# sashapersonxyz/Multi-camera_3D_Pose_Estimation

Hardware: AMD Instinct MI355X
Metric: multi-view frames/sec end-to-end (2-cam HRNet-W32, 17 kpts) at 1/2/4/8 GPUs (higher is better)
Workload: dtype bf16; 1 GPU; BASELINE config 2: 2-cam HRNet-W32 256x192 bf16 (flip test) + batched 4x4 DLT-SVD triangulation; views=2, parallelism=dp1 (frame-sharded)

## Files before the change

multi-camera_3d_pose_estimation_amd/csrc/mfma_tile.h:

```cpp
#pragma once
#include <hip/hip_runtime.h>
#include <cstdint>

namespace mvp {
namespace mfma_tile {

typedef __bf16 bf16x8 __attribute__((ext_vector_type(8)));
typedef float f32x16 __attribute__((ext_vector_type(16)));
typedef __bf16 bf16x2 __attribute__((ext_vector_type(2)));
typedef float f32x2 __attribute__((ext_vector_type(2)));
typedef __attribute__((address_space(3))) void lds_void;
typedef const __attribute__((address_space(1))) void gbl_void;

__device__ __forceinline__ void glds16(const void* src, void* lds_base) {
    __builtin_amdgcn_global_load_lds((gbl_void*)src, (lds_void*)lds_base, 16, 0, 0);
}
__device__ __forceinline__ float relu1_asm(float v) {
    float r;
    asm("v_max_f32 %0, 0, %1" : "=v"(r) : "v"(v));
    return r;
}
__device__ __forceinline__ float relu1(float v) { return __builtin_amdgcn_fmed3f(v, 0.f, __builtin_inff()); }
__device__ __forceinline__ uint32_t pack_bf16x2(float lo, float hi) {
    return __builtin_bit_cast(uint32_t, __builtin_convertvector((f32x2){lo, hi}, bf16x2));
}
__device__ __forceinline__ float lo_bf16(uint32_t u) { return __uint_as_float(u << 16); }
__device__ __forceinline__ float hi_bf16(uint32_t u) { return __uint_as_float(u & 0xffff0000u); }

__host__ __device__ constexpr int row_cout(int r) { return 16 * ((r >> 2) & 1) + 4 * (r >> 3) + (r & 3); }

__device__ __forceinline__ int lane_rank(int r32, int& g2) {
    if (r32 < 4) { g2 = 0; return r32; }
    if (r32 < 12) { g2 = 1; return r32 - 4; }
    if (r32 < 16) { g2 = 0; return r32 - 8; }
    if (r32 < 20) { g2 = 1; return r32 - 8; }
    if (r32 < 28) { g2 = 0; return r32 - 12; }
    g2 = 1;
    return r32 - 16;
}
template <int W, int TH, int NB>
__device__ __forceinline__ int frag_pixel(int f, int r32) {
    int g2;
    const int rank = lane_rank(r32, g2), g = 2 * f + g2;
    if constexpr (W % 16 == 0) {
        return g * 16 + rank;
    } else if constexpr (W == 24 && TH == 16 && NB == 1) {
        if (g < 16) return g * 24 + rank;
        const int k = g - 16;
        return rank < 8 ? k * 24 + 16 + rank : (k + 8) * 24 + 8 + rank;
    } else {
        return f * 32 + r32;
    }
}

__device__ __forceinline__ int lane_grp(int r32) { return (0x96 >> (r32 >> 2)) & 1; }
__device__ __forceinline__ int lane_pos(int r32) { return 4 * (r32 >> 3) + (r32 & 3); }
__device__ __forceinline__ int blk_row(int r32) { return 2 * (r32 >> 3) + lane_grp(r32); }
__device__ __forceinline__ int blk_col(int r32) { return r32 & 3; }

template <int W, int TH, int NB>
__device__ __forceinline__ int frag_pixel_blk(int f, int r32) {
    static_assert(W % 4 == 0 && TH % 8 == 0, "8x4 blocks");
    constexpr int FC = W / 4, FPC = (TH / 8) * FC;
    const int nb = f / FPC, rem = f - nb * FPC, rb = rem / FC, cb = rem - rb * FC;
    return (nb * TH + 8 * rb + blk_row(r32)) * W + 4 * cb + blk_col(r32);
}

}
}
```

multi-camera_3d_pose_estimation_amd/csrc/s2conv.hip:

```cpp
#include <algorithm>
#include <cstdlib>

#include "conv.h"
#include "mfma_tile.h"
#include "mvp_common.h"

namespace mvp {
namespace {

using namespace mfma_tile;

constexpr int kZeroSlots = 4096;

template <int CIN, int H, int W, int TH, int NB, bool WRES, int BM, bool PM_ = false>
struct SCfg {
    static constexpr int NW = 8, NT_THREADS = NW * 64;
    static constexpr int MG = BM / 32, PG = NW / MG;
    static constexpr int NT = 3;
    static constexpr int HO = H / 2, WO = W / 2;
    static constexpr int P = NB * TH * WO;
    static constexpr int NCH = CIN / 16;
    static constexpr int RS = WO + 1, HR = TH + 1;
    static constexpr int PH = HR * RS;
    static constexpr int HS = NB * 4 * PH;
    static constexpr int HT = 2 * HS;
    static constexpr bool PM = PM_;
    static constexpr int QS = PM ? 1 : HS, PS = PM ? 2 : 1;
    static constexpr int WT = 9 * 2 * BM;
    static constexpr int ITEM_SLOTS = HT + (WRES ? 0 : WT);
    static constexpr int PPW = (ITEM_SLOTS + 64 * NW - 1) / (64 * NW);
    static constexpr int BUF = PPW * NW * 1024;
    static constexpr int WPPW = WRES ? (NCH * WT + 64 * NW - 1) / (64 * NW) : 0;
    static constexpr int WOFF = 2 * BUF;
    static constexpr int LDS = 2 * BUF + WPPW * NW * 1024;
    static constexpr int STORES = 2 * NT;
    static_assert(P == PG * NT * 32, "tile = pixel groups x 3 fragments x 32 pixels");
    static_assert(H % 2 == 0 && W % 2 == 0 && HO % TH == 0 && CIN % 16 == 0, "tiling");
    static_assert(LDS <= 160 * 1024, "LDS budget");
    static_assert((QS + (3 * PH + RS + 1) * PS) * 16 < 65536 && (16 * BM + 2 * BM) * 16 < 65536,
                  "ds_read offset range");
    static_assert(STORES < 64 && 2 * PPW < 64, "vmcnt range");
    static_assert(2 * TH + 1 < 256, "row index packing");
};

struct SParams {
    const uint16_t* x;
    const uint16_t* w;
    const float* bias;
    uint16_t* y;
    const uint16_t* zero;
    uint16_t* sink;
    int N, Cout, n_tiles, ncb, relu;
    uint16_t* y1;
    uint16_t* y2;
    int c1, c2, relu1, relu2;
    int img;
};

template <int CIN, int H, int W, int TH, int NB, bool WRES, int BM, bool PM>
__global__ __launch_bounds__(512, 1) void s2conv_kernel(SParams p) {
    using G = SCfg<CIN, H, W, TH, NB, WRES, BM, PM>;
    extern __shared__ __attribute__((aligned(1024))) uint8_t lds[];
    const int tid = threadIdx.x, lane = tid & 63, h = lane >> 5, r32 = lane & 31;
    const int wave = __builtin_amdgcn_readfirstlane(tid >> 6);
    const int mg = wave % G::MG, pg = wave / G::MG;
    if ((int)blockIdx.x >= p.n_tiles) return;
    constexpr int tiles_h = G::HO / TH;

    auto wsrc_off = [&](int ws) {
        const int tq = ws / BM, co = ws - (ws / BM) * BM;
        const int cs = (co & ~31) | row_cout(co & 31);
        return (cs * 9 + (tq >> 1)) * CIN + (tq & 1) * 8;
    };

    constexpr bool SPLIT = !WRES;
    constexpr int NVW = SPLIT ? 2 : 1;
    const bool dma_wave = !SPLIT || wave < 4;
    auto vwave = [&](int v) { return SPLIT ? (wave & 3) + 4 * v : wave; };
    int pk[NVW][G::PPW], po[NVW][G::PPW];
#pragma unroll
    for (int v = 0; v < NVW; v++)
#pragma unroll
    for (int j = 0; j < G::PPW; j++) {
        const int s = (j * G::NW + vwave(v)) * 64 + lane;
        int kind = 0, off = 0, nb = 0, hy = 0;
        if (s < G::HT) {
            const int qh = PM ? s & 1 : s / G::HS, hs = PM ? s >> 1 : s - (s / G::HS) * G::HS;
            nb = hs / (4 * G::PH);
            const int rem = hs - nb * (4 * G::PH);
            const int ph = rem / G::PH, rr = rem - (rem / G::PH) * G::PH;
            const int a = rr / G::RS, b = rr - (rr / G::RS) * G::RS;
            hy = 2 * a + (ph >> 1);
            const int col = 2 * b + (ph & 1) - 1;
            if (col >= 0 && col < W) {
                kind = 1;
                off = ((nb * H + hy - 1) * W + col) * CIN + qh * 8;
            }
        } else if (!WRES && s < G::HT + G::WT) {
            kind = 2;
            off = p.img ? (s - G::HT) * 8 : wsrc_off(s - G::HT);
        }
        pk[v][j] = (kind << 28) | (nb << 8) | hy;
        po[v][j] = off;
    }
    const uint16_t* zl = p.zero + ((wave * 64 + lane) & (kZeroSlots - 1)) * 8;

    auto tile_of = [&](int tile, int& n0, int& ho0, int& cb) {
        cb = tile % p.ncb;
        const int sp = tile / p.ncb;
        n0 = (sp / tiles_h) * NB;
        ho0 = (sp - (sp / tiles_h) * tiles_h) * TH;
    };
    auto issue = [&](int item, int buf) {
        const int tile = blockIdx.x + (item / G::NCH) * gridDim.x, slice = item % G::NCH;
        int n0, ho0, cb;
        tile_of(tile, n0, ho0, cb);
        const uint16_t* xb = p.x + ((long)(n0 * H + 2 * ho0) * W) * CIN + slice * 16;
        const uint16_t* wb =
            p.img ? p.w + (long)(cb * G::NCH + slice) * G::WT * 8 : p.w + (long)cb * BM * 9 * CIN + slice * 16;
        uint8_t* dst = lds + buf * G::BUF;
        if (!dma_wave) return;
#pragma unroll
        for (int v = 0; v < NVW; v++)
#pragma unroll
        for (int j = 0; j < G::PPW; j++) {
            const int vw = vwave(v);
            const int g = pk[v][j], kind = g >> 28, nb = (g >> 8) & 255, hy = g & 255;
            const bool in = kind == 1 && (unsigned)(2 * ho0 + hy - 1) < (unsigned)H && n0 + nb < p.N;
            const uint16_t* src = (!WRES && kind == 2) ? wb + po[v][j] : in ? xb + po[v][j] : zl;
            if (j < G::PPW - 1 || (j * G::NW + vw) * 64 < G::ITEM_SLOTS)
                glds16(src, dst + (j * G::NW + vw) * 1024);
        }
    };

    int bv[G::NT], eoff[G::NT], enb[G::NT];
#pragma unroll
    for (int t = 0; t < G::NT; t++) {
        const int pp = frag_pixel<G::WO, TH, NB>(pg * G::NT + t, r32);
        const int nb = pp / (TH * G::WO), rem = pp - nb * (TH * G::WO);
        const int ty = rem / G::WO, x = rem - (rem / G::WO) * G::WO;
        bv[t] = (h * G::QS + (nb * 4 * G::PH + ty * G::RS + x) * G::PS) * 16;
        eoff[t] = (nb * G::HO + ty) * G::WO + x;
        enb[t] = nb;
    }
    const int av = WRES ? G::WOFF + (h * BM + mg * 32 + r32) * 16 : (G::HT + h * BM + mg * 32 + r32) * 16;

    const int n_items = ((p.n_tiles - 1 - (int)blockIdx.x) / (int)gridDim.x + 1) * G::NCH;
    if (WRES) {
#pragma unroll
        for (int j = 0; j < G::WPPW; j++) {
            const int s = (j * G::NW + wave) * 64 + lane;
            const int slice = s / G::WT;
            const uint16_t* src = s < G::NCH * G::WT ? p.w + slice * 16 + wsrc_off(s - slice * G::WT) : zl;
            glds16(src, lds + G::WOFF + (j * G::NW + wave) * 1024);
        }
    }
    issue(0, 0);
    f32x16 acc[G::NT];
    for (int k = 0; k < n_items; k++) {
        const int buf = k & 1, slice = k % G::NCH;
        const bool first = slice == 0, last = slice == G::NCH - 1;
        if (k == 0 || !first)
            asm volatile("s_waitcnt vmcnt(0)" ::: "memory");
        else
            asm volatile("s_waitcnt vmcnt(%0)" ::"n"(G::STORES) : "memory");
        asm volatile("" ::: "memory");
        __builtin_amdgcn_s_barrier();
        asm volatile("" ::: "memory");
        const int tile = blockIdx.x + (k / G::NCH) * gridDim.x;
        int n0, ho0, cb;
        tile_of(tile, n0, ho0, cb);
        const int cob = cb * BM + mg * 32 + 16 * h;
        if (first) {
            f32x16 b;
#pragma unroll
            for (int j = 0; j < 4; j++) {
                const float4 b4 = *reinterpret_cast<const float4*>(p.bias + cob + 4 * j);
                b[4 * j] = b4.x;
                b[4 * j + 1] = b4.y;
                b[4 * j + 2] = b4.z;
                b[4 * j + 3] = b4.w;
            }
#pragma unroll
            for (int t = 0; t < G::NT; t++) acc[t] = b;
        }
        const bool more = k + 1 < n_items;
        if (more) issue(k + 1, buf ^ 1);
        asm volatile("" ::: "memory");

        const int boff = buf * G::BUF;
        int bva[G::NT];
#pragma unroll
        for (int t = 0; t < G::NT; t++) bva[t] = bv[t] + boff;
        const int ava = WRES ? av + slice * G::WT * 16 : av + boff;
        bf16x8 fa[2], fb[2][G::NT];
        auto load = [&](int tap, bf16x8& a, bf16x8 (&b)[G::NT]) {
            const int dy = tap / 3, dx = tap % 3;
            const int toff = ((dy & 1) * 2 + (dx & 1)) * G::PH + (dy >> 1) * G::RS + (dx >> 1);
            a = *reinterpret_cast<const bf16x8*>(lds + ava + tap * 2 * BM * 16);
#pragma unroll
            for (int t = 0; t < G::NT; t++) b[t] = *reinterpret_cast<const bf16x8*>(lds + bva[t] + toff * G::PS * 16);
        };
        load(0, fa[0], fb[0]);
#pragma unroll
        for (int tap = 0; tap < 9; tap++) {
            const int cur = tap & 1;
            if (tap + 1 < 9) load(tap + 1, fa[cur ^ 1], fb[cur ^ 1]);
            __builtin_amdgcn_sched_barrier(0);
#pragma unroll
            for (int t = 0; t < G::NT; t++)
                acc[t] = __builtin_amdgcn_mfma_f32_32x32x16_bf16(fa[cur], fb[cur][t], acc[t], 0, 0, 0);
            __builtin_amdgcn_sched_barrier(0);
        }

        if (last) {
            const long pix0 = (long)(n0 * G::HO + ho0) * G::WO;
            uint16_t* yb = p.y;
            int cs = p.Cout, cl = cob, rl = p.relu;
            bool cok = true;
            if (cob >= p.Cout) {
                const bool s1 = cob < p.Cout + p.c1;
                yb = s1 ? p.y1 : p.y2;
                cs = s1 ? p.c1 : p.c2;
                cl = s1 ? cob - p.Cout : cob - p.Cout - p.c1;
                rl = s1 ? p.relu1 : p.relu2;
                cok = cob < p.Cout + p.c1 + p.c2;
            }
#pragma unroll
            for (int t = 0; t < G::NT; t++) {
                const bool ok = n0 + enb[t] < p.N && cok;
                uint16_t* yrow = ok ? yb + (pix0 + eoff[t]) * cs + cl : p.sink + lane * 16;
                uint32_t o[8];
#pragma unroll
                for (int e = 0; e < 8; e++) {
                    float v0 = acc[t][2 * e], v1 = acc[t][2 * e + 1];
                    if (rl) {
                        v0 = relu1(v0);
                        v1 = relu1(v1);
                    }
                    o[e] = pack_bf16x2(v0, v1);
                }
                *reinterpret_cast<uint4*>(yrow) = uint4{o[0], o[1], o[2], o[3]};
                *reinterpret_cast<uint4*>(yrow + 8) = uint4{o[4], o[5], o[6], o[7]};
            }
        }
    }
    asm volatile("s_waitcnt vmcnt(0)" ::: "memory");
}

uint16_t* g_s_sink = nullptr;

template <int CIN, int H, int W, int TH, int NB, bool WRES, int BM, bool PM>
void launch_sp_pm(SParams p, hipStream_t s) {
    using G = SCfg<CIN, H, W, TH, NB, WRES, BM, PM>;
    auto kern = s2conv_kernel<CIN, H, W, TH, NB, WRES, BM, PM>;
    static bool attr = false;
    if (!attr) {
        MVP_HIP(hipFuncSetAttribute((const void*)kern, hipFuncAttributeMaxDynamicSharedMemorySize, G::LDS));
        attr = true;
    }
    const int grid = std::min(p.n_tiles, cu_count());
    hipLaunchKernelGGL(kern, dim3(grid), dim3(G::NT_THREADS), G::LDS, s, p);
}

template <int CIN, int H, int W, int TH, int NB, bool WRES, int BM>
void launch_sp(SParams p, hipStream_t s) {
    launch_sp_pm<CIN, H, W, TH, NB, WRES, BM, true>(p, s);
}

template <int CIN, int H, int W, int TH, int NB, bool WRES, int BM>
void launch_s(const ConvLaunch& c, hipStream_t s) {
    using G = SCfg<CIN, H, W, TH, NB, WRES, BM>;
    if (!g_s_sink) MVP_HIP(hipMalloc(&g_s_sink, 64 * 32));
    MVP_REQUIRE(!WRES || c.Cout == BM, "s2conv: resident weights need Cout == BM");
    MVP_REQUIRE(c.Cout % BM == 0, "s2conv: Cout %d not a multiple of %d", c.Cout, BM);
    MVP_REQUIRE(c.Cin == CIN && c.H == H && c.W == W, "s2conv: plane mismatch");
    const long tiles = (long)((c.N + NB - 1) / NB) * (G::HO / TH) * (c.Cout / BM);
    MVP_REQUIRE(tiles < (1L << 30), "s2conv: too many tiles");
    const bool img = !WRES && BM == 128 && c.w_img != nullptr;
    SParams p{c.x, img ? c.w_img : c.w, c.bias, c.y, conv_zero_region(), g_s_sink, c.N, c.Cout, (int)tiles,
              c.Cout / BM, c.relu, nullptr, nullptr, 0, 0, 0, 0, img ? 1 : 0};
    launch_sp<CIN, H, W, TH, NB, WRES, BM>(p, s);
}

void init_s() {
    if (!g_s_sink) MVP_HIP(hipMalloc(&g_s_sink, 64 * 32));
}

}

bool s2conv_multi_supported(int H, int W, int Cin, int total_cout) {
    return H == 64 && W == 48 && Cin == 32 && total_cout <= 128;
}

void launch_s2conv_multi(const S2Multi& m, hipStream_t s) {
    MVP_REQUIRE(m.n_out >= 1 && m.n_out <= 3, "s2conv_multi: %d outputs", m.n_out);
    int tot = 0;
    for (int i = 0; i < m.n_out; i++) {
        MVP_REQUIRE(m.cout[i] % 32 == 0 && m.cout[i] > 0, "s2conv_multi: cout %d", m.cout[i]);
        tot += m.cout[i];
    }
    MVP_REQUIRE(s2conv_multi_supported(m.H, m.W, m.Cin, tot), "s2conv_multi: unsupported plane");
    init_s();
    using G = SCfg<32, 64, 48, 8, 1, true, 128>;
    const long tiles = (long)m.N * (G::HO / 8);
    SParams p{m.x, m.w, m.bias, m.y[0], conv_zero_region(), g_s_sink, m.N, m.cout[0], (int)tiles, 1, m.relu[0],
              m.n_out > 1 ? m.y[1] : nullptr, m.n_out > 2 ? m.y[2] : nullptr, m.n_out > 1 ? m.cout[1] : 0,
              m.n_out > 2 ? m.cout[2] : 0, m.n_out > 1 ? m.relu[1] : 0, m.n_out > 2 ? m.relu[2] : 0, 0};
    if (tiles == 0) return;
    launch_sp<32, 64, 48, 8, 1, true, 128>(p, s);
    MVP_HIP(hipGetLastError());
}

void launch_s2conv(const ConvLaunch& c, hipStream_t s) {
    MVP_REQUIRE(c.ks == 3 && c.stride == 2 && !c.out_f32_nchw && !c.res && !c.x2, "s2conv: not a plain 3x3/s2 conv");
    const int ci = c.Cin, co = c.Cout, h = c.H, w = c.W;
    const bool p24 = h == 32 && w == 24 && co == 128;
    const bool p12 = h == 16 && w == 12 && co % 128 == 0;
    if (h == 64 && w == 48 && co == 64 && ci == 32)
        launch_s<32, 64, 48, 16, 1, true, 64>(c, s);
    else if (p24 && ci == 32)
        launch_s<32, 32, 24, 16, 1, true, 128>(c, s);
    else if (p24 && ci == 64)
        launch_s<64, 32, 24, 16, 1, false, 128>(c, s);
    else if (p12 && ci == 32)
        launch_s<32, 16, 12, 8, 4, false, 128>(c, s);
    else if (p12 && ci == 64)
        launch_s<64, 16, 12, 8, 4, false, 128>(c, s);
    else if (p12 && ci == 128)
        launch_s<128, 16, 12, 8, 4, false, 128>(c, s);
    else
        fail(MVP_ERR_ARG, "s2conv: unsupported plane %d -> %d @ %dx%d", ci, co, h, w);
    MVP_HIP(hipGetLastError());
}

}
```

Measured before the change: 12920 frames/s.

## Triple-buffer halo loads and stage bias in LDS for stride-2 conv

Splits the per-item DMA into separate halo and weight transfers, so the halo input can use a three-deep LDS ring when it fits while weights stay double-buffered. The waits allow a prefetch that is further ahead to stay in flight. Bias is also copied into LDS once per block and read with ds_read instead of global loads at each tile start. This costs more LDS and tighter Cout limits (at most 2 channel blocks), and the finer vmcnt accounting risks ordering errors.

```diff
diff --git a/multi-camera_3d_pose_estimation_amd/csrc/mfma_tile.h b/multi-camera_3d_pose_estimation_amd/csrc/mfma_tile.h
--- a/multi-camera_3d_pose_estimation_amd/csrc/mfma_tile.h
+++ b/multi-camera_3d_pose_estimation_amd/csrc/mfma_tile.h
@@ -14,6 +14,25 @@
 
 __device__ __forceinline__ void glds16(const void* src, void* lds_base) {
     __builtin_amdgcn_global_load_lds((gbl_void*)src, (lds_void*)lds_base, 16, 0, 0);
+}
+template <int N>
+__device__ __forceinline__ void wait_vm() {
+    static_assert(N >= 0 && N < 64, "vmcnt is 6 bits");
+    asm volatile("s_waitcnt vmcnt(%0)" ::"n"(N) : "memory");
+}
+typedef float f32x4 __attribute__((ext_vector_type(4)));
+__device__ __forceinline__ f32x16 lds_read16_unseen(const void* p) {
+    f32x4 b[4];
+    asm volatile(
+        "ds_read_b128 %0, %4\n\tds_read_b128 %1, %4 offset:16\n\t"
+        "ds_read_b128 %2, %4 offset:32\n\tds_read_b128 %3, %4 offset:48\n\ts_waitcnt lgkmcnt(0)"
+        : "=&v"(b[0]), "=&v"(b[1]), "=&v"(b[2]), "=&v"(b[3])
+        : "v"((uint32_t)(size_t)(lds_void*)p)
+        : "memory");
+    f32x16 r;
+#pragma unroll
+    for (int e = 0; e < 16; e++) r[e] = b[e >> 2][e & 3];
+    return r;
 }
 __device__ __forceinline__ float relu1_asm(float v) {
     float r;
diff --git a/multi-camera_3d_pose_estimation_amd/csrc/s2conv.hip b/multi-camera_3d_pose_estimation_amd/csrc/s2conv.hip
--- a/multi-camera_3d_pose_estimation_amd/csrc/s2conv.hip
+++ b/multi-camera_3d_pose_estimation_amd/csrc/s2conv.hip
@@ -27,19 +27,26 @@
     static constexpr bool PM = PM_;
     static constexpr int QS = PM ? 1 : HS, PS = PM ? 2 : 1;
     static constexpr int WT = 9 * 2 * BM;
-    static constexpr int ITEM_SLOTS = HT + (WRES ? 0 : WT);
-    static constexpr int PPW = (ITEM_SLOTS + 64 * NW - 1) / (64 * NW);
-    static constexpr int BUF = PPW * NW * 1024;
+    static constexpr int NDW = WRES ? NW : 4;
+    static constexpr int HP = (HT + 63) / 64, WP = WRES ? 0 : WT / 64;
+    static constexpr int HPW = (HP + NDW - 1) / NDW, HPW_MIN = HP / NDW, WPW = WP / NDW;
+    static constexpr int HBUF = HP * 1024, WBUF = WP * 1024;
     static constexpr int WPPW = WRES ? (NCH * WT + 64 * NW - 1) / (64 * NW) : 0;
-    static constexpr int WOFF = 2 * BUF;
-    static constexpr int LDS = 2 * BUF + WPPW * NW * 1024;
+    static constexpr int WBYTES = WRES ? WPPW * NW * 1024 : 2 * WBUF;
+    static constexpr int NCB = WRES ? 1 : 2;
+    static constexpr int BIAS_BYTES = NCB * BM * 4;
+    static constexpr int DEPTH = 3 * HBUF + WBYTES + BIAS_BYTES <= 160 * 1024 ? 3 : 2;
+    static constexpr int WOFF = DEPTH * HBUF, BIAS_OFF = WOFF + WBYTES;
+    static constexpr int LDS = BIAS_OFF + BIAS_BYTES;
+    static constexpr int AHEAD = DEPTH == 3 ? HPW_MIN : 0;
     static constexpr int STORES = 2 * NT;
     static_assert(P == PG * NT * 32, "tile = pixel groups x 3 fragments x 32 pixels");
     static_assert(H % 2 == 0 && W % 2 == 0 && HO % TH == 0 && CIN % 16 == 0, "tiling");
     static_assert(LDS <= 160 * 1024, "LDS budget");
     static_assert((QS + (3 * PH + RS + 1) * PS) * 16 < 65536 && (16 * BM + 2 * BM) * 16 < 65536,
                   "ds_read offset range");
-    static_assert(STORES < 64 && 2 * PPW < 64, "vmcnt range");
+    static_assert(WRES || WT % (64 * NDW) == 0, "weight slices are whole pieces, the same number on every DMA wave");
+    static_assert(AHEAD + STORES < 64, "vmcnt range");
     static_assert(2 * TH + 1 < 256, "row index packing");
 };
 
@@ -73,16 +80,17 @@
         return (cs * 9 + (tq >> 1)) * CIN + (tq & 1) * 8;
     };
 
-    constexpr bool SPLIT = !WRES;
-    constexpr int NVW = SPLIT ? 2 : 1;
-    const bool dma_wave = !SPLIT || wave < 4;
-    auto vwave = [&](int v) { return SPLIT ? (wave & 3) + 4 * v : wave; };
-    int pk[NVW][G::PPW], po[NVW][G::PPW];
-#pragma unroll
-    for (int v = 0; v < NVW; v++)
-#pragma unroll
-    for (int j = 0; j < G::PPW; j++) {
-        const int s = (j * G::NW + vwave(v)) * 64 + lane;
+    const bool dma_wave = wave < G::NDW;
+    const int dw = wave & (G::NDW - 1);
+    int pk[G::HPW], po[G::HPW], pw[G::WPW > 0 ? G::WPW : 1];
+#pragma unroll
+    for (int j = 0; j < G::WPW; j++) {
+        const int ws = (j * G::NDW + dw) * 64 + lane;
+        pw[j] = p.img ? ws * 8 : wsrc_off(ws);
+    }
+#pragma unroll
+    for (int j = 0; j < G::HPW; j++) {
+        const int s = (j * G::NDW + dw) * 64 + lane;
         int kind = 0, off = 0, nb = 0, hy = 0;
         if (s < G::HT) {
             const int qh = PM ? s & 1 : s / G::HS, hs = PM ? s >> 1 : s - (s / G::HS) * G::HS;
@@ -96,12 +104,9 @@
                 kind = 1;
                 off = ((nb * H + hy - 1) * W + col) * CIN + qh * 8;
             }
-        } else if (!WRES && s < G::HT + G::WT) {
-            kind = 2;
-            off = p.img ? (s - G::HT) * 8 : wsrc_off(s - G::HT);
-        }
-        pk[v][j] = (kind << 28) | (nb << 8) | hy;
-        po[v][j] = off;
+        }
+        pk[j] = (kind << 28) | (nb << 8) | hy;
+        po[j] = off;
     }
     const uint16_t* zl = p.zero + ((wave * 64 + lane) & (kZeroSlots - 1)) * 8;
 
@@ -111,26 +116,31 @@
         n0 = (sp / tiles_h) * NB;
         ho0 = (sp - (sp / tiles_h) * tiles_h) * TH;
     };
-    auto issue = [&](int item, int buf) {
+    auto issue_halo = [&](int item, int slot) {
         const int tile = blockIdx.x + (item / G::NCH) * gridDim.x, slice = item % G::NCH;
         int n0, ho0, cb;
         tile_of(tile, n0, ho0, cb);
         const uint16_t* xb = p.x + ((long)(n0 * H + 2 * ho0) * W) * CIN + slice * 16;
+        uint8_t* dst = lds + slot * G::HBUF;
+        if (!dma_wave) return;
+#pragma unroll
+        for (int j = 0; j < G::HPW; j++) {
+            const int g = pk[j], kind = g >> 28, nb = (g >> 8) & 255, hy = g & 255;
+            const bool in = kind == 1 && (unsigned)(2 * ho0 + hy - 1) < (unsigned)H && n0 + nb < p.N;
+            if (j < G::HPW_MIN || j * G::NDW + dw < G::HP)
+                glds16(in ? xb + po[j] : zl, dst + (j * G::NDW + dw) * 1024);
+        }
+    };
+    auto issue_weights = [&](int item, int slot) {
+        const int tile = blockIdx.x + (item / G::NCH) * gridDim.x, slice = item % G::NCH;
+        int n0, ho0, cb;
+        tile_of(tile, n0, ho0, cb);
         const uint16_t* wb =
             p.img ? p.w + (long)(cb * G::NCH + slice) * G::WT * 8 : p.w + (long)cb * BM * 9 * CIN + slice * 16;
-        uint8_t* dst = lds + buf * G::BUF;
-        if (!dma_wave) return;
-#pragma unroll
-        for (int v = 0; v < NVW; v++)
-#pragma unroll
-        for (int j = 0; j < G::PPW; j++) {
-            const int vw = vwave(v);
-            const int g = pk[v][j], kind = g >> 28, nb = (g >> 8) & 255, hy = g & 255;
-            const bool in = kind == 1 && (unsigned)(2 * ho0 + hy - 1) < (unsigned)H && n0 + nb < p.N;
-            const uint16_t* src = (!WRES && kind == 2) ? wb + po[v][j] : in ? xb + po[v][j] : zl;
-            if (j < G::PPW - 1 || (j * G::NW + vw) * 64 < G::ITEM_SLOTS)
-                glds16(src, dst + (j * G::NW + vw) * 1024);
-        }
+        uint8_t* dst = lds + G::WOFF + slot * G::WBUF + dw * 1024;
+        if (WRES || !dma_wave) return;
+#pragma unroll
+        for (int j = 0; j < G::WPW; j++) glds16(wb + pw[j], dst + j * G::NDW * 1024);
     };
 
     int bv[G::NT], eoff[G::NT], enb[G::NT];
@@ -143,9 +153,12 @@
         eoff[t] = (nb * G::HO + ty) * G::WO + x;
         enb[t] = nb;
     }
-    const int av = WRES ? G::WOFF + (h * BM + mg * 32 + r32) * 16 : (G::HT + h * BM + mg * 32 + r32) * 16;
+    const int av = G::WOFF + (h * BM + mg * 32 + r32) * 16;
 
     const int n_items = ((p.n_tiles - 1 - (int)blockIdx.x) / (int)gridDim.x + 1) * G::NCH;
+    for (int i = tid; i < p.ncb * BM; i += G::NT_THREADS)
+        reinterpret_cast<float*>(lds + G::BIAS_OFF)[i] = p.bias[i];
+    asm volatile("s_waitcnt lgkmcnt(0)" ::: "memory");
     if (WRES) {
 #pragma unroll
         for (int j = 0; j < G::WPPW; j++) {
@@ -155,15 +168,26 @@
             glds16(src, lds + G::WOFF + (j * G::NW + wave) * 1024);
         }
     }
-    issue(0, 0);
+    issue_halo(0, 0);
+    issue_weights(0, 0);
+    if (G::DEPTH == 3 && n_items > 1) issue_halo(1, 1);
     f32x16 acc[G::NT];
+    int hs = 0;
     for (int k = 0; k < n_items; k++) {
         const int buf = k & 1, slice = k % G::NCH;
         const bool first = slice == 0, last = slice == G::NCH - 1;
-        if (k == 0 || !first)
-            asm volatile("s_waitcnt vmcnt(0)" ::: "memory");
-        else
-            asm volatile("s_waitcnt vmcnt(%0)" ::"n"(G::STORES) : "memory");
+        const bool more = k + 1 < n_items;
+        if (k == 0 || !first) {
+            if (more)
+                wait_vm<G::AHEAD>();
+            else
+                wait_vm<0>();
+        } else {
+            if (more)
+                wait_vm<G::AHEAD + G::STORES>();
+            else
+                wait_vm<G::STORES>();
+        }
         asm volatile("" ::: "memory");
         __builtin_amdgcn_s_barrier();
         asm volatile("" ::: "memory");
@@ -172,27 +196,21 @@
         tile_of(tile, n0, ho0, cb);
         const int cob = cb * BM + mg * 32 + 16 * h;
         if (first) {
-            f32x16 b;
-#pragma unroll
-            for (int j = 0; j < 4; j++) {
-                const float4 b4 = *reinterpret_cast<const float4*>(p.bias + cob + 4 * j);
-                b[4 * j] = b4.x;
-                b[4 * j + 1] = b4.y;
-                b[4 * j + 2] = b4.z;
-                b[4 * j + 3] = b4.w;
-            }
+            const f32x16 b = lds_read16_unseen(lds + G::BIAS_OFF + cob * 4);
 #pragma unroll
             for (int t = 0; t < G::NT; t++) acc[t] = b;
         }
-        const bool more = k + 1 < n_items;
-        if (more) issue(k + 1, buf ^ 1);
         asm volatile("" ::: "memory");
-
-        const int boff = buf * G::BUF;
+        if (more) issue_weights(k + 1, buf ^ 1);
+        if (k + G::DEPTH - 1 < n_items) issue_halo(k + G::DEPTH - 1, hs == 0 ? G::DEPTH - 1 : hs - 1);
+        asm volatile("" ::: "memory");
+
+        const int boff = hs * G::HBUF;
         int bva[G::NT];
 #pragma unroll
         for (int t = 0; t < G::NT; t++) bva[t] = bv[t] + boff;
-        const int ava = WRES ? av + slice * G::WT * 16 : av + boff;
+        const int ava = WRES ? av + slice * G::WT * 16 : av + buf * G::WBUF;
+        hs = hs == G::DEPTH - 1 ? 0 : hs + 1;
         bf16x8 fa[2], fb[2][G::NT];
         auto load = [&](int tap, bf16x8& a, bf16x8 (&b)[G::NT]) {
             const int dy = tap / 3, dx = tap % 3;
@@ -273,7 +291,7 @@
     using G = SCfg<CIN, H, W, TH, NB, WRES, BM>;
     if (!g_s_sink) MVP_HIP(hipMalloc(&g_s_sink, 64 * 32));
     MVP_REQUIRE(!WRES || c.Cout == BM, "s2conv: resident weights need Cout == BM");
-    MVP_REQUIRE(c.Cout % BM == 0, "s2conv: Cout %d not a multiple of %d", c.Cout, BM);
+    MVP_REQUIRE(c.Cout % BM == 0 && c.Cout / BM <= G::NCB, "s2conv: Cout %d not 1..%d blocks of %d", c.Cout, G::NCB, BM);
     MVP_REQUIRE(c.Cin == CIN && c.H == H && c.W == W, "s2conv: plane mismatch");
     const long tiles = (long)((c.N + NB - 1) / NB) * (G::HO / TH) * (c.Cout / BM);
     MVP_REQUIRE(tiles < (1L << 30), "s2conv: too many tiles");
```

After: 12990 frames/s (median of 6 runs). No clear change (+0.6%).
